# schmidtjonathan/pnmol-experiments

Hardware: AMD Instinct MI355X
Metric: filter steps/sec, 1D heat N=512 nu=2 (white-noise EK1 predict+update) (higher is better)
Workload: dtype f64; 1 GPU; 1-D heat equation, N=512 mesh, IWP(nu=2) EK1, Dirichlet, dt=2^-7, one problem per GPU (kappa sweep), D=1536, m=514; steps_in_one_call=4975, valid=True, problems_per_gpu=1

## Files before the change

### include/pnmol_hip.h

```cpp
#ifndef PNMOL_HIP_H
#define PNMOL_HIP_H

#ifdef __cplusplus
extern "C" {
#endif

typedef struct pnmol_ctx pnmol_ctx;
typedef struct pnmol_filter pnmol_filter;
typedef struct pnmol_state pnmol_state;
typedef struct pnmol_samples pnmol_samples;
typedef struct pnmol_bridge pnmol_bridge;

int pnmol_abi_version(void);
int pnmol_device_count(int* count);
int pnmol_ctx_create(int device, pnmol_ctx** out);
int pnmol_ctx_destroy(pnmol_ctx* ctx);
int pnmol_ctx_synchronize(pnmol_ctx* ctx);
const char* pnmol_last_error(pnmol_ctx* ctx);

int pnmol_fd_solve_batched(pnmol_ctx* ctx, const double* gram_nss, const double* lk_ns, const double* llk_n, int N, int s,
                           double* weights_ns, double* uncertainty_n);
int pnmol_cholesky_lower(pnmol_ctx* ctx, const double* A_nn, int n, double* L_nn);

typedef struct pnmol_filter_desc {
    int d;
    int num_derivatives;
    int nB;
    const double* L;
    const double* B;
    const double* E_sqrtm;
    const double* R_sqrtm;
    const double* Gamma;
    int d_state;
    int dtype;
    const double* K;
} pnmol_filter_desc;

int pnmol_filter_create(pnmol_ctx* ctx, const pnmol_filter_desc* desc, pnmol_filter** out);
int pnmol_filter_destroy(pnmol_filter* f);
int pnmol_filter_sweep_layout(const pnmol_filter* f, int* kernel, int* xcd_home);

int pnmol_filter_set_error_model(pnmol_filter* f, double dt, const double* Sq_inv,
                                 const double* Sq_diag);
int pnmol_filter_prepare_error_model(pnmol_filter* f, double dt);

int pnmol_filter_predict_mean(pnmol_filter* f, const pnmol_state* in, double dt, double* m_at_d);
int pnmol_filter_set_operator(pnmol_filter* f, const double* M_dds, const double* shift_d);
int pnmol_filter_set_operator_diagonal(pnmol_filter* f, const double* jdiag_d, const double* shift_d);

#define PNMOL_REACTION_MAXDEG 7
typedef struct pnmol_reaction {
    int deg_p, deg_a, deg_b;
    double p[PNMOL_REACTION_MAXDEG + 1], a[PNMOL_REACTION_MAXDEG + 1], b[PNMOL_REACTION_MAXDEG + 1];
} pnmol_reaction;
int pnmol_filter_set_reaction(pnmol_filter* f, const pnmol_reaction* r);
int pnmol_filter_linearize(pnmol_filter* f, const pnmol_state* in, double dt);

#define PNMOL_SYSTEM_MAXCOMP  4
#define PNMOL_SYSTEM_MAXTERMS 8
typedef struct pnmol_monomial    { double coef; int pow[PNMOL_SYSTEM_MAXCOMP]; } pnmol_monomial;
typedef struct pnmol_system_poly { int nterms; pnmol_monomial term[PNMOL_SYSTEM_MAXTERMS]; } pnmol_system_poly;
typedef struct pnmol_reaction_system {
    int ncomp;
// ... 82 lines not shown
```

### pnmol-experiments_amd/csrc/pnmol_hip.hip

```cpp
#include <hip/hip_runtime.h>

#include <algorithm>
#include <chrono>
#include <cmath>
#include <cstdio>
#include <cstdlib>
#include <cstring>
#include <string>
#include <utility>
#include <atomic>
#include <vector>

#include "pnmol_hip.h"
#include "pnmol_internal.hpp"

namespace {

constexpr int TLD = NB + 1;
typedef double d4 __attribute__((ext_vector_type(4)));

struct MeasModel {
    const int* ell_col;
    const double* ell_val;
    int w, d, m, dp, mp;
    double c0, c1;
};

constexpr int HW = 4;

struct HRow {
    int idx[HW + 1];
    double cf[HW + 1];
};

__device__ __forceinline__ void h_row_load(const MeasModel& mm, int i, HRow& r) {
    r.idx[0] = (i < mm.d) ? mm.dp + i : 0;
    r.cf[0] = (i < mm.d) ? mm.c1 : 0.0;
// ... 1675 lines not shown
                    L.seen[0] = got;
                }
                __syncthreads();
                const int got = L.seen[0];
                if (got < 0) break;
                if (got == 0) continue;
                ksplit_partial(L.sP[w], Xh, F + ((long)t * NB + fr) * ld + 8 * fk, 0, kh, ld, w, l);
                __syncthreads();
                double* hs = hs_scratch + ((long)H * CB + t) * NB * NB;
#pragma unroll
                for (int r = 0; r < 4; ++r)
                    wt_st(&hs[(wr * 16 + fk + 4 * r) * NB + colC],
                          (L.sP[0][offC + 4 * r * TLD] + L.sP[1][offC + 4 * r * TLD]) +
                              (L.sP[2][offC + 4 * r * TLD] + L.sP[3][offC + 4 * r * TLD]));
                drain_vmem();
                __syncthreads();
                if (tid == 0) flag_st(cl, 2);
            }
        }
    }
}

constexpr int RL_REP = 8;
constexpr int S_SPLIT_FROM = 11, S_SPLIT_H = 9;
__host__ __device__ inline int s_split_count(int CB, bool xl) { return (xl && CB > S_SPLIT_FROM) ? CB - S_SPLIT_FROM : 0; }
constexpr int W_SPLIT_H = 11;
#ifndef PNMOL_W_SPLIT
#define PNMOL_W_SPLIT 0
#endif
__host__ __device__ inline int w_split_count(int RT, int CB) {
    const int RBW = RT - 2 * CB - 1;
    return (PNMOL_W_SPLIT && RBW > 0 && CB > W_SPLIT_H + 1) ? RBW : 0;
}
struct RlFlags {
    int frow, fabort, fxcc, ffeed, fdiag, fnew, fcol, fdiagL, fnewL, frowL, CBp, total;
};
__host__ __device__ inline RlFlags rl_flags(int RT, int CB) {
    const int RTp = (RT + 31) / 32 * 32, CBp = (CB + 31) / 32 * 32;
    RlFlags f;
    f.CBp = CBp;
    f.frow = 0;
    f.fabort = RTp;
    f.fxcc = RTp + 16;
    f.ffeed = RTp + 32;
    f.fdiag = f.ffeed + CBp;
    f.fnew = f.fdiag + RL_REP * CBp;
    f.fcol = f.fnew + RL_REP * CBp;
    f.fdiagL = f.fcol + RL_REP * CBp;
    f.fnewL = f.fdiagL + CBp;
    f.frowL = f.fnewL + CBp;
    f.total = f.frowL + CBp;
    return f;
}
__device__ __forceinline__ int xcc_id() { return __builtin_amdgcn_s_getreg((3 << 11) | 20) & 15; }
struct WaveWait {
    bool dead;
// ... 287 lines not shown
                TileRegs tx;
                tile_regs_from_lds(tx, C.sX, l);
                tile_regs_store<0>(tx, rF, orgX, ld, l);
                drain_vmem();
                if (l == 0) l2_flag_st(rflags, fl.fnewL + J, 1);
                tile_regs_store<16>(tl, rlinv, (unsigned)(J * NB * NB * 8), NB, l);
                tile_regs_store<16>(tx, rF, orgX, ld, l);
                drain_vmem();
                if (l < RL_REP) flag_st(fdiag_all + l * CBp + J, 1);
                if (l < RL_REP) flag_st(fnew_all + l * CBp + J, 1);
            } else {
                wt_rows_from_lds<8>(rF, orgX, ld, C.sX, 0, l);
                drain_vmem();
                if (l < RL_REP) flag_st(fnew_all + l * CBp + J, 1);
            }
        }
    }
    if (w == 2)
        diag4_output(&C.d4[(CB - 1) & 1], l, F + ((long)(CB - 1) * NB) * ld + (long)(CB - 1) * NB, ld, info, (CB - 1) * NB,
                     C.sd[(CB - 1) & 1], smax, pivtol);
    if (l == 0 && ww.dead) atomicMin(info, -2);
}

template <int N, bool FUSED, int MAXT, bool XL>
__global__ __launch_bounds__(256) void k_sweep_rl(const double* __restrict__ G, double* F, double* Linv, int ld, int CB,
                                                  int RT, int* flags, int* info_base, const int* __restrict__ ctr,
                                                  DowndateArgs dd, double* feed, int lenient, int home) {
    __shared__ __attribute__((aligned(16))) union {
        SweepLds L;
        ChainLds C;
    } lds;
    SweepLds& L = lds.L;
    __shared__ __attribute__((aligned(16))) double bulk_ring[4][RING + 2][16 * NB];
    const int tid = threadIdx.x, l = tid & 63, w = __builtin_amdgcn_readfirstlane(tid >> 6);
    const int wr = w >> 1, wc = w & 1, fr = l & 15, fk = l >> 4;
    const RlFlags fl = rl_flags(RT, CB);
    int* frow = flags + fl.frow;
    int* fabort = flags + fl.fabort;
    int* ffeed = flags + fl.ffeed;
    const int* fdiag = flags + fl.fdiag + (blockIdx.x % RL_REP) * fl.CBp;
    const int* fnew = flags + fl.fnew + (blockIdx.x % RL_REP) * fl.CBp;
    const int* fcol = flags + fl.fcol + (blockIdx.x % RL_REP) * fl.CBp;
    int* info = info_base + (*ctr - 1);
    const int bx = XL ? (int)blockIdx.x - home : (int)blockIdx.x;
    if (bx < 0) return;
    if (bx == 0) {
        sweep_chain_role<XL>(lds.C, G, F, Linv, ld, CB, flags, fl, info, feed, lenient, tid, l, w);
        return;
    }
    int I, part = 0;
    if constexpr (XL) {
        const int nsplit = s_split_count(CB, true);
        const int b = bx, nslot = 8 * (CB - 1 + nsplit) + 1;
        if (b < nslot) {
            if (b % 8 != 0) return;
            const int sidx = b / 8;
            if (sidx < CB) {
                I = sidx;
                part = (nsplit > 0 && I >= S_SPLIT_FROM) ? 1 : 0;
            } else {
                I = S_SPLIT_FROM + (sidx - CB);
                part = 2;
            }
        } else {
            if (b % 8 == 0) return;
            const int q = b - nslot;
            I = CB + q - (q + 1) / 8;
        }
    } else {
        I = bx - 1;
    }
#ifdef PNMOL_SWEEP_STAMP
    if (tid == 0) L.stamp_id = part == 1 ? 200 + I : 1 + I;
#endif
    {
        const int zb = RT - CB - 1;
        if (I >= CB && I <= zb) I = (I == CB) ? zb : I - 1;
    }
    const int nwsplit = w_split_count(RT, CB);
    if (I >= RT && I < RT + nwsplit) {
        I = CB + (I - RT);
        part = 2;
    } else if (I >= RT) {
        I -= nwsplit;
        if constexpr (FUSED) {
            if (tid == 0) {
                L.dead = 0, L.seen[0] = 0;
                __builtin_amdgcn_fence(__ATOMIC_ACQUIRE, "agent");
            }
            __syncthreads();
            SWEEP_STAMP(0);
            sweep_downdate_role<N, true>(L, dd, F, ld, CB, CB, frow, fabort, info, I - RT, tid, l, w, *ctr - 1);
        }
        return;
    } else if (nwsplit > 0 && I >= CB && I < RT - CB - 1) {
        part = 1;
    }
    const bool chain = I < CB;
    if (chain && I == 0) return;
    if (tid == 0) {
        L.dead = 0, L.pub = 0, L.pubcnt = part == 2 ? 4 * (I < CB ? S_SPLIT_H : W_SPLIT_H) : 0, L.rdiag = 0, L.rnew = 0, L.rcol = 0, L.rzb = 0;
        L.seen[0] = 0;
        __builtin_amdgcn_fence(__ATOMIC_ACQUIRE, "agent");
    }
    __syncthreads();
    SWEEP_STAMP(0);

    const long rowC = (long)I * NB + wr * 16 + fk;
    const int colC = wc * 16 + fr;
    const int offC = (wr * 16 + fk) * TLD + colC;
    const bool feeds = chain && part != 1;
    const int hsplit = chain ? S_SPLIT_H : W_SPLIT_H;
    const int t0 = part == 2 ? hsplit : 0;
    const int last = part == 1 ? hsplit - 1 : (chain ? I - 2 : CB - 1);
    const int ntiles = part == 1 ? hsplit : (chain ? I : CB);
    d4 n[MAXT];
#pragma unroll
    for (int t = 0; t < MAXT; ++t)
        if (t0 + t < ntiles) {
#pragma unroll
            for (int r = 0; r < 4; ++r) n[t][r] = -G[(rowC + 4 * r) * ld + (long)(t0 + t) * NB + colC];
        }
    d4 accD = {0, 0, 0, 0};
    if (feeds) {
#pragma unroll
        for (int r = 0; r < 4; ++r) {
            const int rl = wr * 16 + fk + 4 * r, cl = colC;
            accD[r] = -G[((long)I * NB + (rl >= cl ? rl : cl)) * ld + (long)I * NB + (rl >= cl ? cl : rl)];
        }
    }
    WaveWait ww{false};
    int known_diag = 0, known_new = 0, known_col = 0;
    const __amdgpu_buffer_rsrc_t rF = wt_rsrc(F), rfeed = wt_rsrc(feed), rflags = wt_rsrc(flags);
    const double* ringw = &bulk_ring[w][0][0];
    const unsigned ring0 = __builtin_amdgcn_readfirstlane((unsigned)(size_t)ringw);
    int roff[4], roffL[4];
#pragma unroll
    for (int c = 0; c < 4; ++c) {
        const int row = 4 * c + (l >> 4);
        roff[c] = (wc * 16 + row) * ld + 2 * ((l & 15) ^ row);
        roffL[c] = (wc * 16 + row) * NB + 2 * ((l & 15) ^ row);
    }
#ifndef PNMOL_EAGER_TILES
#define PNMOL_EAGER_TILES 6
#endif
    constexpr int EAGER_TILES = PNMOL_EAGER_TILES;
    bool pre_b0 = false;
    if constexpr (FUSED) {
        const int RBW = RT - 2 * CB - 1, zb = CB + RBW;
        if (!chain && I > zb) {
            double bq[8] = {0, 0, 0, 0, 0, 0, 0, 0};
            if (dd.va.Sqinv != nullptr) rows8_dot(dd.va.Sqinv, (long)(I - zb - 1) * NB + 8 * w, ld, dd.va.z, bq, l);
            if (l == 0) {
#pragma unroll
                for (int q = 0; q < 8; ++q) L.sd[8 * w + q] = bq[q];
            }
        }
    }
    bool local = false;
    if constexpr (XL) {
        if (chain) {
            if (tid == 0) {
                int v = 0;
                for (int spins = 0; spins < 4096 && (v = flag_ld(flags + fl.fxcc)) == 0; ++spins) __builtin_amdgcn_s_sleep(1);
                L.seen[0] = (v == 1 + xcc_id());
            }
            __syncthreads();
            local = L.seen[0] != 0;
            if (local) fdiag = flags + fl.fdiagL, fnew = flags + fl.fnewL;
        }
    }
    Frag8 ax;
    auto flag_tile = [&](int t) {
        drain_vmem();
        int lastw = 0;
        if (l == 0) lastw = __hip_atomic_fetch_add(&L.pubcnt, 1, __ATOMIC_RELAXED, __HIP_MEMORY_SCOPE_WORKGROUP) == 4 * t + 3;
        if (__builtin_amdgcn_readfirstlane(lastw)) {
            if (l == 0) flag_st(frow + I, t + 1);
            if (XL && chain && l == 0) {
                if (local) l2_flag_st(rflags, fl.frowL + I, t + 1);
                else flag_st(flags + fl.frowL + I, t + 1);
            }
            if (chain && l < RL_REP)
                __hip_atomic_fetch_add(flags + fl.fcol + l * fl.CBp + t, 1, __ATOMIC_RELAXED, __HIP_MEMORY_SCOPE_AGENT);
        }
    };
    if (part == 2) {
        const int* fsrc = (XL && local) ? flags + fl.frowL : frow;
        for (int k = 0; k < t0; ++k) {
            if (chain) {
                if (k + 1 < t0) {
                    relay_progress_min(fsrc + t0, I - t0 + 1, k + 1, known_col, &L.rcol, fabort, ww, w, l);
                } else {
                    relay_progress(fnew, CB - 1, [](int) { return 1; }, t0, known_new, &L.rnew, fabort, ww, w, l);
                    relay_progress_min(fsrc + t0 + 1, I - t0, t0, known_col, &L.rcol, fabort, ww, w, l);
                }
            } else {
                relay_progress(fnew, CB - 1, [](int) { return 1; }, k + 1, known_new, &L.rnew, fabort, ww, w, l);
                relay_progress(fcol, CB - 1, [CB](int q) { return CB - 2 - q; }, k + 1, known_col, &L.rcol, fabort, ww, w, l);
                relay_wait_ge(frow + I, k + 1, &L.rzb, k + 1, fabort, ww, w);
            }
            Frag8 bx;
            frag_ld(ax, F + ((long)I * NB + wr * 16 + fr) * ld + (long)k * NB + 8 * fk);
            frag_ld(bx, F + ((long)I * NB + wc * 16 + fr) * ld + (long)k * NB + 8 * fk);
#pragma unroll
            for (int u0 = 0; u0 < 8; u0 += 4) {
                Frag8 b[4];
#pragma unroll
                for (int q = 0; q < 4; ++q)
                    if (t0 + u0 + q < ntiles)
                        frag_ld(b[q], F + ((long)(t0 + u0 + q) * NB + wc * 16 + fr) * ld + (long)k * NB + 8 * fk);
#pragma unroll
                for (int q = 0; q < 4; ++q)
                    if (t0 + u0 + q < ntiles) {
#pragma unroll
                        for (int s = 0; s < 8; ++s)
                            n[u0 + q] = __builtin_amdgcn_mfma_f64_16x16x4f64(ax.v[s], b[q].v[s], n[u0 + q], 0, 0, 0);
                    }
            }
            if (chain) {
#pragma unroll
                for (int s = 0; s < 8; ++s) accD = __builtin_amdgcn_mfma_f64_16x16x4f64(ax.v[s], bx.v[s], accD, 0, 0, 0);
            }
// ... 642 lines not shown
inline bool fused_loop(const pnmol_filter* f) {
    return f->sweep_mode == 2 && f->n <= 3 && f->fuse_predict != 0 && !f->has_reaction;
}

inline bool sweep_rl_enabled() {
    static const int on = [] {
        const char* e = std::getenv("PNMOL_HIP_SWEEP_RL");
        return e ? std::atoi(e) : 1;
    }();
    return on != 0;
}
inline int sweep_xl_mode() {
    static const int mode = [] {
        const char* e = std::getenv("PNMOL_HIP_SWEEP_XL");
        return e ? (std::atoi(e) != 0 ? 1 : 0) : -1;
    }();
    return mode;
}
constexpr int MAX_DEVICES = 64;
std::atomic<int> live_rl_filters[MAX_DEVICES];
template <int N, bool FUSED>
void launch_sweep(unsigned grid, hipStream_t st, const double* G, double* F, double* Linv, int ld, int CB, int RT, int* flags,
                  int* info, const int* ctr, const DowndateArgs& dd, int* claim, double* hs, int lenient, int home,
                  bool wskip = false) {
    const bool xl = home >= 0;
    const unsigned rgrid = grid + (unsigned)w_split_count(RT, CB);
    unsigned xgrid = 8u * (unsigned)(CB - 1 + s_split_count(CB, true)) + 1u;
    for (unsigned left = rgrid - (unsigned)CB; left > 0; ++xgrid)
        if (xgrid % 8u != 0u) --left;
    xgrid += (unsigned)(xl ? home : 0);
    if (sweep_rl_enabled() && CB <= 9) {
        if (xl) k_sweep_rl<N, FUSED, 9, true><<<xgrid, 256, 0, st>>>(G, F, Linv, ld, CB, RT, flags, info, ctr, dd, hs, lenient, home);
        else k_sweep_rl<N, FUSED, 9, false><<<rgrid + 1, 256, 0, st>>>(G, F, Linv, ld, CB, RT, flags, info, ctr, dd, hs, lenient, home);
    } else if (sweep_rl_enabled() && CB <= 17) {
        if (xl) k_sweep_rl<N, FUSED, 17, true><<<xgrid, 256, 0, st>>>(G, F, Linv, ld, CB, RT, flags, info, ctr, dd, hs, lenient, home);
        else k_sweep_rl<N, FUSED, 17, false><<<rgrid + 1, 256, 0, st>>>(G, F, Linv, ld, CB, RT, flags, info, ctr, dd, hs, lenient, home);
    }
    else
        k_sweep<N, FUSED><<<grid, 256, 0, st>>>(G, F, Linv, ld, CB, RT, flags, info, ctr, dd, claim, hs, lenient, wskip ? 1 : 0);
}

inline bool short_last_panel() {
    static const int on = [] {
        const char* e = std::getenv("PNMOL_HIP_SHORT_LAST");
        return e ? std::atoi(e) : 1;
    }();
    return on != 0;
}
template <int N>
int launch_step(pnmol_filter* f, const double* Pin, const double* min, double frame_dt, double dt, double* Pout,
                double* mout, double* varout, bool record, StepKind kind) {
    pnmol_ctx* ctx = f->ctx;
    hipStream_t st = ctx->stream;
    IwpConsts c = f->iwp;
    for (int a = 0; a < f->n; ++a) {
        const double so = frame_dt == 0.0 ? 1.0 : nordsieck_scale(f->nu, a, frame_dt);
        c.ts[a] = so / nordsieck_scale(f->nu, a, dt);
    }
    MeasModel mm{f->ell_col, f->ell_val, f->ellw, f->d, f->m, f->dp, f->mp,
// ... 8 lines not shown
        if (f->ellw > HW && f->sweep_mode != 0) {
            k_front<<<dim3((mp + 255) / 256, (unsigned)Dp), 256, 0, st>>>(f->Ppred, f->G, f->rdiag, f->Rdense, mm, Dp, f->p32);
            k_front_s<<<dim3((mp + 255) / 256, (unsigned)mp), 256, 0, st>>>(f->G, f->rdiag, f->Rdense, mm);
        } else {
            k_front<<<dim3((mp + 255) / 256, (unsigned)(Dp + mp + (f->sweep_mode == 0 ? mp : 0))), 256, 0, st>>>(
                f->Ppred, f->G, f->rdiag, f->Rdense, mm, Dp, f->p32);
        }
    }
    const long rowI0 = (long)mp + Dp + NB;
    const double* W = f->F + (long)mp * mp;
    const bool have_sq = (f->Sqinv != nullptr && f->sq_dt == dt);
    VecArgs va{f->mpred, f->F + ((long)mp + Dp) * mp, f->F + rowI0 * mp, f->zbuf, have_sq ? f->Sqinv : nullptr,
               mout, f->part};
    const int nreal = f->m - NB * (f->CB - 1);
    DowndateArgs dd{f->Ppred, Pout, varout, dp, 0, va, kind == STEP_FULL ? nullptr : f->Ppred, f->Kg, f->last_ctr, {}, {}, f->p32,
                    (nreal < 8 && short_last_panel()) ? nreal : 0};
    std::memcpy(dd.A1, f->iwp.A1, sizeof(dd.A1));
    std::memcpy(dd.Q1, f->iwp.Q1, sizeof(dd.Q1));
    if (f->sweep_mode == 2) {
        const int t32 = dp / NB, pairs = t32 * (t32 + 1) / 2;
        dd.vrows = 0;
        if constexpr (N <= 3)
            launch_sweep<N, true>(f->RT + pairs, st, f->G, f->F, f->Linv, mp, f->CB, f->RT, f->flags, f->info, f->ctr, dd,
                                  f->flags + f->RT + f->CB + 1, f->hs_scratch, f->p32 ? 2 : 0, f->xcd_home);
    } else {
        if (f->sweep_mode == 1) {
            if (f->w_gemm) {
                launch_sweep<N, false>(2 * f->CB + 1, st, f->G, f->F, f->Linv, mp, f->CB, f->RT, f->flags, f->info, f->ctr, dd,
                                       f->flags + f->RT + f->CB + 1, f->hs_scratch, f->p32 ? 2 : 0, f->xcd_home, true);
                const int nI = (int)(Dp / BDT), nt = nI * (mp / BDT);
                k_w_gemm<<<8 * ((nt + 7) / 8), 256, 0, st>>>(f->G + (long)mp * mp, f->F + rowI0 * mp, f->F + (long)mp * mp, mp, nI, nt);
            } else
            launch_sweep<N, false>(f->RT, st, f->G, f->F, f->Linv, mp, f->CB, f->RT, f->flags, f->info, f->ctr, dd,
                                   f->flags + f->RT + f->CB + 1, f->hs_scratch, f->p32 ? 2 : 0, f->xcd_home);
        } else {
            k_diag0<<<1, 128, 0, st>>>(f->G, f->F, f->Linv, mp, f->info, f->sdiag, f->ctr);
            for (int j = 0; j < f->CB; ++j) {
                const int nrb = f->RT - (j + 1);
                const int ncb = f->CB - 1 - j > 0 ? f->CB - 1 - j : 1;
                k_panel<<<dim3(nrb, ncb), 256, 0, st>>>(f->G, f->F, f->Linv, mp, j, f->CB, f->RBS, f->info, f->sdiag, f->ctr);
            }
        }
        const int tiles = dp / 16;
        const int vrows = (int)(((Dp + mp + 3) / 4 + tiles - 1) / tiles);
        if (f->dd_big) {
            const int T = (int)(Dp / BDT), nt = T * (T + 1) / 2;
            if (f->p32)
// ... 538 lines not shown
    if (const char* gc = std::getenv("PNMOL_HIP_GRAPH_CHUNK")) f->graph_chunk = std::atoi(gc) / 2 * 2;
    if (const char* e = std::getenv("PNMOL_HIP_SWEEP")) f->sweep_mode = std::atoi(e);
    if (f->sweep_mode == 2 && n > 3) f->sweep_mode = 1;
    {
        const char* e = std::getenv("PNMOL_HIP_DD_BIG");
        const bool fits = f->Dp % BDT == 0 && f->mp % BDK == 0 && f->sweep_mode >= 1 && (!f->p32 || f->sweep_mode == 2);
        const bool want = e ? std::atoi(e) != 0 : (f->Dp >= 8192 && f->CB > 17);
        if (fits && want) {
            f->dd_big = 1;
            f->sweep_mode = 1;
            const char* g = std::getenv("PNMOL_HIP_W_GEMM");
            f->w_gemm = (g ? std::atoi(g) != 0 : 1) && f->mp % BDT == 0 && f->CB > 17;
        }
    }
    {
        static std::atomic<int> next_home[MAX_DEVICES];
        const bool rl = sweep_rl_enabled() && f->CB <= 17 && f->sweep_mode >= 1;
        if (rl) {
            const int dv = ctx->device % MAX_DEVICES;
            const int others = live_rl_filters[dv].fetch_add(1);
            f->counted = true;
            const bool xl = sweep_xl_mode() < 0 ? others == 0 : sweep_xl_mode() == 1;
            f->xcd_home = xl ? next_home[dv].fetch_add(1) % 8 : -1;
        }
    }
    FCHK(hipMalloc(&f->sdiag, sizeof(double) * (mp + 1)));
    f->nflags = std::max({f->RT + f->CB + 1 + f->CB * f->CB, rl_flags(f->RT, f->CB).total,
                          rl_flags((int)(f->Dp / NB) + 1, (int)(f->Dp / NB) + 1).total});
    FCHK(hipMalloc(&f->flags, sizeof(int) * f->nflags));
    FCHK(hipMemset(f->flags, 0, sizeof(int) * f->nflags));
    FCHK(hipMalloc(&f->hs_scratch, sizeof(double) * (size_t)std::max(f->CB * f->CB, 2 * f->CB + 2) * NB * NB));
    if (const char* e = std::getenv("PNMOL_HIP_FUSE_PREDICT")) f->fuse_predict = std::atoi(e);
    FCHK(hipMalloc(&f->last_ctr, sizeof(int)));
    FCHK(hipMemset(f->last_ctr, 0, sizeof(int)));
    FCHK(hipMalloc(&f->tickets, sizeof(int)));
    FCHK(hipMemset(f->tickets, 0, sizeof(int)));
    if (f->p32 && f->sweep_mode != 2 && !f->dd_big) {
        ctx->err = "pnmol_filter_create: dtype = fp32 covariance needs the fused sweep (num_derivatives <= 2, PNMOL_HIP_SWEEP unset)";
        return fail(-1);
    }
    FCHK(hipMemcpy(f->ell_col, ecol.data(), sizeof(int) * ecol.size(), hipMemcpyHostToDevice));
    FCHK(hipMemcpy(f->ell_val, eval.data(), sizeof(double) * eval.size(), hipMemcpyHostToDevice));
    {
        std::vector<int> slot((size_t)mp, 0);
        f->base_has_diag = 1;
        for (int i = 0; i < d; ++i) {
// ... 69 lines not shown
    pnmol_dense_free_ws(f);
    pnmol_observe_free_ws(f);
    pnmol_reaction_free_ws(f);
    if (f->ev0) hipEventDestroy(f->ev0);
    if (f->ev1) hipEventDestroy(f->ev1);
    delete f;
    return 0;
}

int pnmol_filter_dims(const pnmol_filter* f, int* d, int* n, int* m, int* dp, int* mp) {
    if (!f) return -1;
    if (d) *d = f->d;
    if (n) *n = f->n;
    if (m) *m = f->m;
    if (dp) *dp = f->dp;
    if (mp) *mp = f->mp;
    return 0;
}

int pnmol_filter_sweep_layout(const pnmol_filter* f, int* kernel, int* xcd_home) {
    if (!f) return -1;
    if (kernel) *kernel = f->sweep_mode == 0 ? 0 : (sweep_rl_enabled() && f->CB <= 17 ? 2 : 1);
    if (xcd_home) *xcd_home = f->xcd_home;
    return 0;
}

int pnmol_filter_set_error_model(pnmol_filter* f, double dt, const double* Sq_inv, const double* Sq_diag) {
    if (!f || !Sq_inv || !Sq_diag || !(dt > 0.0)) return -1;
    pnmol_ctx* ctx = f->ctx;
    HIPCHK(ctx, hipSetDevice(ctx->device));
    const int m = f->m, mp = f->mp;
    std::vector<double> pad((size_t)mp * mp, 0.0);
    for (int i = 0; i < m; ++i) std::memcpy(&pad[(size_t)i * mp], Sq_inv + (size_t)i * m, sizeof(double) * m);
    HIPCHK(ctx, hipStreamSynchronize(ctx->stream));
    if (!f->Sqinv) HIPCHK(ctx, hipMalloc(&f->Sqinv, sizeof(double) * pad.size()));
    HIPCHK(ctx, hipMemcpy(f->Sqinv, pad.data(), sizeof(double) * pad.size(), hipMemcpyHostToDevice));
    f->sqdiag.assign(Sq_diag, Sq_diag + m);
    f->sq_dt = dt;
    drop_graphs(f);
    return 0;
}

int pnmol_filter_prepare_error_model(pnmol_filter* f, double dt) {
    if (!f || !(dt > 0.0)) return -1;
    pnmol_ctx* ctx = f->ctx;
    HIPCHK(ctx, hipSetDevice(ctx->device));
// ... 619 lines not shown
```

### pnmol-experiments_amd/csrc/pnmol_internal.hpp

```cpp
#pragma once
#include <hip/hip_runtime.h>

#include <algorithm>
#include <atomic>
#include <cmath>
#include <string>
#include <vector>

#include "pnmol_hip.h"

constexpr int NB = 32;
constexpr int MAXN = 4;

namespace {
struct IwpConsts {
    double A1[MAXN * MAXN];
    double Q1[MAXN * MAXN];
    double ts[MAXN];
};
}

#define HIPCHK(ctx, call)                                                                        \
    do {                                                                                         \
        hipError_t e__ = (call);                                                                 \
// ... 35 lines not shown
    int qp = 0;
    SweepWs sweep;
    double* dev = nullptr;
    std::vector<double> host;
};

struct pnmol_filter {
    pnmol_ctx* ctx = nullptr;
    int d = 0, n = 0, nu = 0, nB = 0, m = 0, dp = 0, mp = 0, CB = 0, RBS = 0, RBW = 0, RT = 0, ellw = 0;
    int* tickets = nullptr;
    int* last_ctr = nullptr;
    int fuse_predict = 1;
    int* flags = nullptr;
    int nflags = 0;
    double* hs_scratch = nullptr;
    int w_gemm = 0;
    int dd_big = 0;
    int sweep_mode = 2;
    int ds = 0;
    bool counted = false;
    bool registered = false;
    std::atomic<int> states{0};
    int xcd_home = -1;
    int p32 = 0;
    size_t psz = 8;
    long Dp = 0;
    IwpConsts iwp{};
    int* ell_col = nullptr;
    double* ell_val = nullptr;
    int* ell_col_base = nullptr;
    double* ell_val_base = nullptr;
    int* ell_diag_slot = nullptr;
    int base_w = 0, base_has_diag = 0;
    int ell_is_base = 1;
    double* h_op = nullptr;
    double* h_op_dev = nullptr;
    hipEvent_t ev_op = nullptr;
    double *Kg = nullptr, *rdiag = nullptr, *Rdense = nullptr, *shift = nullptr;
    double *G = nullptr, *F = nullptr, *Linv = nullptr, *Ppred = nullptr, *mpred = nullptr, *zbuf = nullptr;
    double *var = nullptr, *Sqinv = nullptr, *rec = nullptr, *part = nullptr, *sdiag = nullptr;
    int* info = nullptr;
    std::vector<double> sqdiag;
    double* Qfull = nullptr;
    int* one = nullptr;
    int* info_err = nullptr;
    double sq_dt = -1.0;
// ... 156 lines not shown
```

### pnmol-experiments_amd/pnmol/_hip.py

```python

import ctypes
import os
import pathlib

import numpy as np


_c_double_p = ctypes.POINTER(ctypes.c_double)
_HERE = pathlib.Path(__file__).resolve().parent
LIB_PATH = pathlib.Path(os.environ.get("PNMOL_HIP_LIB", _HERE.parent / "lib" / "libpnmol_hip.so"))


class PnmolHipError(RuntimeError):
    """A call into libpnmol_hip.so failed."""


class StepOut(ctypes.Structure):
    _fields_ = [
        ("t_new", ctypes.c_double),
        ("diffusion_squared_local", ctypes.c_double),
        ("sigma2_whitened", ctypes.c_double),
        ("error_sigma2", ctypes.c_double),
        ("info", ctypes.c_int),
    ]
# ... 69 lines not shown
    "pnmol_samples_create": (ctypes.c_int, [_vp, ctypes.c_int, ctypes.POINTER(_vp)]),
    "pnmol_samples_destroy": (ctypes.c_int, [_vp]),
    "pnmol_samples_draw": (ctypes.c_int, [_vp, _vp, _c_double_p, ctypes.c_ulonglong, ctypes.c_ulonglong, ctypes.c_double]),
    "pnmol_samples_step_back": (ctypes.c_int, [_vp, _vp, ctypes.c_double, _c_double_p, ctypes.c_ulonglong, ctypes.c_ulonglong,
                                               ctypes.c_double]),
    "pnmol_samples_interpolate": (ctypes.c_int, [_vp, _vp, _vp, ctypes.c_double, _c_double_p, ctypes.c_ulonglong,
                                                 ctypes.c_ulonglong, ctypes.c_double]),
    "pnmol_samples_clone": (ctypes.c_int, [_vp, ctypes.POINTER(_vp)]),
    "pnmol_samples_get": (ctypes.c_int, [_vp, _c_double_p]),
    "pnmol_samples_get_time": (ctypes.c_int, [_vp, _c_double_p]),
    "pnmol_sample_noise": (ctypes.c_int, [_vp, ctypes.c_ulonglong, ctypes.c_ulonglong, ctypes.c_int, ctypes.c_int,
                                          _c_double_p]),
    "pnmol_filter_steps": (ctypes.c_int, [_vp, _vp, ctypes.c_int, ctypes.c_double, _c_double_p, _c_double_p,
                                          ctypes.POINTER(StepOut)]),
    "pnmol_filter_steps_begin": (ctypes.c_int, [_vp, _vp, ctypes.c_int, ctypes.c_double]),
    "pnmol_filter_steps_end": (ctypes.c_int, [_vp, _vp, _c_double_p, _c_double_p, ctypes.POINTER(StepOut)]),
    "pnmol_filter_prepare_steps": (ctypes.c_int, [_vp, _vp, ctypes.c_int, ctypes.c_double]),
    "pnmol_filter_last_steps_ms": (ctypes.c_int, [_vp, ctypes.POINTER(ctypes.c_float)]),
    "pnmol_filter_prepare_error_model": (ctypes.c_int, [_vp, ctypes.c_double]),
    "pnmol_filter_debug_read": (ctypes.c_int, [_vp, ctypes.c_int, _c_double_p, ctypes.c_long]),
    "pnmol_filter_debug_poison": (ctypes.c_int, [_vp]),
    "pnmol_filter_dims": (ctypes.c_int, [_vp] + [ctypes.POINTER(ctypes.c_int)] * 5),
    "pnmol_filter_sweep_layout": (ctypes.c_int, [_vp] + [ctypes.POINTER(ctypes.c_int)] * 2),
    "pnmol_qr_r": (ctypes.c_int, [_vp, _c_double_p, ctypes.c_int, ctypes.c_int, _c_double_p]),
    "pnmol_qr_last_ms": (ctypes.c_int, [ctypes.POINTER(ctypes.c_float)]),
    "pnmol_sqrt_propagate_cholesky_factor": (ctypes.c_int, [_vp, _c_double_p, ctypes.c_int, ctypes.c_int, _c_double_p,
                                                             ctypes.c_int, _c_double_p]),
    "pnmol_sqrt_update": (ctypes.c_int, [_vp, _c_double_p, ctypes.c_int, ctypes.c_int, _c_double_p, _c_double_p,
                                         _c_double_p, _c_double_p, _c_double_p]),
    "pnmol_sqrt_filter_create": (ctypes.c_int, [_vp, ctypes.POINTER(FilterDesc), ctypes.POINTER(_vp)]),
    "pnmol_sqrt_filter_destroy": (ctypes.c_int, [_vp]),
    "pnmol_sqrt_filter_set_state": (ctypes.c_int, [_vp, ctypes.c_double, _c_double_p, _c_double_p]),
    "pnmol_sqrt_filter_get_state": (ctypes.c_int, [_vp, _c_double_p, _c_double_p, _c_double_p]),
    "pnmol_sqrt_filter_predict_mean": (ctypes.c_int, [_vp, ctypes.c_double, _c_double_p]),
    "pnmol_sqrt_filter_set_operator": (ctypes.c_int, [_vp, _c_double_p, _c_double_p]),
    "pnmol_sqrt_filter_prepare_error_model": (ctypes.c_int, [_vp, ctypes.c_double]),
    "pnmol_sqrt_filter_step": (ctypes.c_int, [_vp, ctypes.c_double, ctypes.POINTER(StepOut), _c_double_p]),
    "pnmol_sqrt_filter_steps": (ctypes.c_int, [_vp, ctypes.c_int, ctypes.c_double, _c_double_p, _c_double_p,
                                               ctypes.POINTER(StepOut)]),
    "pnmol_sqrt_filter_last_steps_ms": (ctypes.c_int, [_vp, ctypes.POINTER(ctypes.c_float)]),
    "pnmol_sqrt_update_no_meascov": (ctypes.c_int, [_vp, _c_double_p, ctypes.c_int, ctypes.c_int, _c_double_p,
                                                    _c_double_p, _c_double_p, _c_double_p]),
}

_lib = None


def load_library():
    global _lib
    if _lib is None:
        if not LIB_PATH.exists():
            raise PnmolHipError(
                f"{LIB_PATH} not found: build it with `python __graft_entry__.py` (hipcc --offload-arch=gfx950). "
                "pnmol has no CPU fallback for the filter step."
            )
        lib = ctypes.CDLL(str(LIB_PATH))
        for name, (res, args) in SYMBOLS.items():
            fn = getattr(lib, name)
            fn.restype, fn.argtypes = res, args
        _lib = lib
    return _lib


def _dp(a):
    return a.ctypes.data_as(_c_double_p)


def _f64(a, shape=None):
    a = np.ascontiguousarray(np.asarray(a, dtype=np.float64))
    if shape is not None and a.shape != shape:
        raise ValueError(f"expected shape {shape}, got {a.shape}")
    return a


class Context:

    _cache = {}

    def __init__(self, device=0):
        self.lib = load_library()
# ... 119 lines not shown
        self._live_samples = {}
        self._live_bridges = {}

    def __del__(self):
        live = getattr(self, "_live", None)
        while live:
            _, sh = live.popitem()
            self.lib.pnmol_state_destroy(sh)
        live = getattr(self, "_live_samples", None)
        while live:
            _, sh = live.popitem()
            self.lib.pnmol_samples_destroy(sh)
        live = getattr(self, "_live_bridges", None)
        while live:
            _, sh = live.popitem()
            self.lib.pnmol_bridge_destroy(sh)
        h, self.handle = getattr(self, "handle", None), None
        if h:
            self.lib.pnmol_filter_destroy(h)

    def sweep_layout(self):
        k, x = ctypes.c_int(0), ctypes.c_int(0)
        self.lib.pnmol_filter_sweep_layout(self.handle, ctypes.byref(k), ctypes.byref(x))
        return {"kernel": ("per_panel", "k_sweep", "k_sweep_rl")[k.value], "xcd_home": x.value}

    def dims(self):
        v = [ctypes.c_int(0) for _ in range(5)]
        self.lib.pnmol_filter_dims(self.handle, *[ctypes.byref(x) for x in v])
        return dict(zip(("d", "n", "m", "dp", "mp"), (x.value for x in v)))

    def prepare_error_model(self, dt):
        self.ctx.check(self.lib.pnmol_filter_prepare_error_model(self.handle, float(dt)), "pnmol_filter_prepare_error_model")
        self.error_model_dt = float(dt)

    def set_error_model(self, dt, Sq_inv, Sq_diag):
        a, b = _f64(Sq_inv, (self.m, self.m)), _f64(Sq_diag, (self.m,))
        self.ctx.check(self.lib.pnmol_filter_set_error_model(self.handle, float(dt), _dp(a), _dp(b)),
                       "pnmol_filter_set_error_model")
        self.error_model_dt = float(dt)

    def new_state(self):
        return State(self)

    def new_samples(self, num_samples):
        return Samples(self, num_samples)

    def predict_mean(self, state_in, dt):
# ... 367 lines not shown
```

Baseline: 7940 steps/s.

## Add paired W-tail sweep roles and skip leading zero tiles in bottom rows

Moves the sweep block-to-role mapping into a shared layout header and adds an optional tail role, where one workgroup handles two trailing W rows beyond a split point h. It also lets rows below the zero band skip their leading structurally-zero tiles, writing zeros directly instead of accumulating them. The tail split is off by default and is enabled by an environment variable. This adds layout complexity and new flag protocols that could deadlock or mis-order if they are wrong.

```diff
diff --git a/include/pnmol_hip.h b/include/pnmol_hip.h
--- a/include/pnmol_hip.h
+++ b/include/pnmol_hip.h
@@ -39,6 +39,7 @@
 int pnmol_filter_create(pnmol_ctx* ctx, const pnmol_filter_desc* desc, pnmol_filter** out);
 int pnmol_filter_destroy(pnmol_filter* f);
 int pnmol_filter_sweep_layout(const pnmol_filter* f, int* kernel, int* xcd_home);
+int pnmol_filter_sweep_tail(const pnmol_filter* f, int* h, int* rows_per_tail, int* tails);
 
 int pnmol_filter_set_error_model(pnmol_filter* f, double dt, const double* Sq_inv,
                                  const double* Sq_diag);
diff --git a/pnmol-experiments_amd/csrc/pnmol_hip.hip b/pnmol-experiments_amd/csrc/pnmol_hip.hip
--- a/pnmol-experiments_amd/csrc/pnmol_hip.hip
+++ b/pnmol-experiments_amd/csrc/pnmol_hip.hip
@@ -13,6 +13,7 @@
 
 #include "pnmol_hip.h"
 #include "pnmol_internal.hpp"
+#include "pnmol_sweep_layout.hpp"
 
 namespace {
 
@@ -1734,16 +1735,6 @@
 }
 
 constexpr int RL_REP = 8;
-constexpr int S_SPLIT_FROM = 11, S_SPLIT_H = 9;
-__host__ __device__ inline int s_split_count(int CB, bool xl) { return (xl && CB > S_SPLIT_FROM) ? CB - S_SPLIT_FROM : 0; }
-constexpr int W_SPLIT_H = 11;
-#ifndef PNMOL_W_SPLIT
-#define PNMOL_W_SPLIT 0
-#endif
-__host__ __device__ inline int w_split_count(int RT, int CB) {
-    const int RBW = RT - 2 * CB - 1;
-    return (PNMOL_W_SPLIT && RBW > 0 && CB > W_SPLIT_H + 1) ? RBW : 0;
-}
 struct RlFlags {
     int frow, fabort, fxcc, ffeed, fdiag, fnew, fcol, fdiagL, fnewL, frowL, CBp, total;
 };
@@ -2077,10 +2068,165 @@
     if (l == 0 && ww.dead) atomicMin(info, -2);
 }
 
+template <int TT>
+__device__ __forceinline__ void sweep_tail_role(SweepLds& L, const double* __restrict__ G, double* F, const double* Linv, int ld,
+                                                int CB, int RT, int* flags, const RlFlags& fl, const int* fdiag, const int* fnew,
+                                                const int* fcol, int* info, const VecArgs& va, int h, int I0, int I1, int tid,
+                                                int l, int w) {
+    int* frow = flags + fl.frow;
+    int* fabort = flags + fl.fabort;
+    const int wr = w >> 1, wc = w & 1, fr = l & 15, fk = l >> 4;
+    const int colC = wc * 16 + fr, offC = (wr * 16 + fk) * TLD + colC;
+    const bool two = I1 >= 0;
+    const int IB = two ? I1 : I0;
+    const int zb = RT - CB - 1, nt = CB - h;
+    d4 nA[TT], nB[TT];
+#pragma unroll
+    for (int u = 0; u < TT; ++u)
+        if (u < nt) {
+#pragma unroll
+            for (int r = 0; r < 4; ++r) {
+                nA[u][r] = -G[((long)I0 * NB + wr * 16 + fk + 4 * r) * ld + (long)(h + u) * NB + colC];
+                nB[u][r] = -G[((long)IB * NB + wr * 16 + fk + 4 * r) * ld + (long)(h + u) * NB + colC];
+            }
+        }
+    for (int rr = 0; rr < 2; ++rr) {
+        const int Ir = rr ? IB : I0;
+        if (Ir > zb) {
+            double bq[8] = {0, 0, 0, 0, 0, 0, 0, 0};
+            if (va.Sqinv != nullptr) rows8_dot(va.Sqinv, (long)(Ir - zb - 1) * NB + 8 * w, ld, va.z, bq, l);
+            if (l == 0) {
+#pragma unroll
+                for (int q = 0; q < 8; ++q) L.sP[1][32 * rr + 8 * w + q] = bq[q];
+            }
+        }
+    }
+    WaveWait ww{false};
+    int known_diag = 0, known_new = 0, known_col = 0;
+    const __amdgpu_buffer_rsrc_t rF = wt_rsrc(F);
+    for (int k = 0; k < h; ++k) {
+        relay_progress(fnew, CB - 1, [](int) { return 1; }, k + 1, known_new, &L.rnew, fabort, ww, w, l);
+        relay_progress(fcol, CB - 1, [CB](int q) { return CB - 2 - q; }, k + 1, known_col, &L.rcol, fabort, ww, w, l);
+        relay_wait_ge(frow + I0, k + 1, &L.rzb, 2 * k + 1, fabort, ww, w);
+        relay_wait_ge(frow + IB, k + 1, &L.rzb, 2 * k + 2, fabort, ww, w);
+        Frag8 a0, a1;
+        frag_ld(a0, F + ((long)I0 * NB + wr * 16 + fr) * ld + (long)k * NB + 8 * fk);
+        frag_ld(a1, F + ((long)IB * NB + wr * 16 + fr) * ld + (long)k * NB + 8 * fk);
+#pragma unroll
+        for (int u0 = 0; u0 < TT; u0 += 4) {
+            Frag8 b[4];
+#pragma unroll
+            for (int q = 0; q < 4; ++q)
+                if (u0 + q < nt) frag_ld(b[q], F + ((long)(h + u0 + q) * NB + wc * 16 + fr) * ld + (long)k * NB + 8 * fk);
+#pragma unroll
+            for (int q = 0; q < 4; ++q)
+                if (u0 + q < nt) {
+#pragma unroll
+                    for (int s = 0; s < 8; ++s)
+                        nA[u0 + q] = __builtin_amdgcn_mfma_f64_16x16x4f64(a0.v[s], b[q].v[s], nA[u0 + q], 0, 0, 0);
+#pragma unroll
+                    for (int s = 0; s < 8; ++s)
+                        nB[u0 + q] = __builtin_amdgcn_mfma_f64_16x16x4f64(a1.v[s], b[q].v[s], nB[u0 + q], 0, 0, 0);
+                    mfma_result_guard();
+                }
+        }
+        mfma_result_guard();
+    }
+    auto flag_tile = [&](int t) {
+        drain_vmem();
+        int lastw = 0;
+        if (l == 0) lastw = __hip_atomic_fetch_add(&L.pubcnt, 1, __ATOMIC_RELAXED, __HIP_MEMORY_SCOPE_WORKGROUP) == 4 * t + 3;
+        if (__builtin_amdgcn_readfirstlane(lastw) && l == 0) {
+            flag_st(frow + I0, t + 1);
+            if (two) flag_st(frow + I1, t + 1);
+        }
+    };
+#pragma unroll
+    for (int r = 0; r < 4; ++r) {
+        L.sS[0][offC + 4 * r * TLD] = -nA[0][r];
+        L.sS[1][offC + 4 * r * TLD] = -nB[0][r];
+    }
+    __syncthreads();
+    for (int j = h; j < CB; ++j) {
+        relay_progress(fdiag, CB, [](int) { return 1; }, j + 1, known_diag, &L.rdiag, fabort, ww, w, l);
+        Frag8 bl;
+        frag_ld(bl, Linv + (long)j * NB * NB + (wc * 16 + fr) * NB + 8 * fk);
+        d4 x0 = {0, 0, 0, 0}, x1 = {0, 0, 0, 0};
+#pragma unroll
+        for (int s = 0; s < 8; ++s)
+            x0 = __builtin_amdgcn_mfma_f64_16x16x4f64(L.sS[0][(wr * 16 + fr) * TLD + 8 * fk + s], bl.v[s], x0, 0, 0, 0);
+#pragma unroll
+        for (int s = 0; s < 8; ++s)
+            x1 = __builtin_amdgcn_mfma_f64_16x16x4f64(L.sS[1][(wr * 16 + fr) * TLD + 8 * fk + s], bl.v[s], x1, 0, 0, 0);
+        mfma_result_guard();
+#pragma unroll
+        for (int r = 0; r < 4; ++r) {
+            L.sX[offC + 4 * r * TLD] = x0[r];
+            L.sP[0][offC + 4 * r * TLD] = x1[r];
+        }
+        __syncthreads();
+        wt_rows_from_lds<2>(rF, (unsigned)((((long)I0 * NB) * ld + (long)j * NB) * 8), ld, L.sX, 8 * w, l);
+        if (two) wt_rows_from_lds<2>(rF, (unsigned)((((long)I1 * NB) * ld + (long)j * NB) * 8), ld, L.sP[0], 8 * w, l);
+        const int cnt = CB - 1 - j;
+        if (cnt > 0) {
+            Frag8 a0, a1;
+#pragma unroll
+            for (int s = 0; s < 8; ++s) {
+                a0.v[s] = L.sX[(wr * 16 + fr) * TLD + 8 * fk + s];
+                a1.v[s] = L.sP[0][(wr * 16 + fr) * TLD + 8 * fk + s];
+            }
+            relay_progress(fnew, CB - 1, [](int) { return 1; }, j + 1, known_new, &L.rnew, fabort, ww, w, l);
+            relay_progress(fcol, CB - 1, [CB](int q) { return CB - 2 - q; }, j + 1, known_col, &L.rcol, fabort, ww, w, l);
+            const double* Lt = F + (long)j * NB + ((long)j * NB + wc * 16 + fr) * ld + 8 * fk;
+#pragma unroll
+            for (int u0 = 1; u0 < TT; u0 += 4) {
+                Frag8 b[4];
+#pragma unroll
+                for (int q = 0; q < 4; ++q)
+                    if (u0 + q < TT && u0 + q <= cnt) frag_ld(b[q], Lt + (long)(u0 + q) * NB * ld);
+                if (u0 == 1) flag_tile(j);
+#pragma unroll
+                for (int q = 0; q < 4; ++q)
+                    if (u0 + q < TT && u0 + q <= cnt) {
+                        d4 ea = nA[u0 + q], eb = nB[u0 + q];
+#pragma unroll
+                        for (int s = 0; s < 8; ++s) ea = __builtin_amdgcn_mfma_f64_16x16x4f64(a0.v[s], b[q].v[s], ea, 0, 0, 0);
+#pragma unroll
+                        for (int s = 0; s < 8; ++s) eb = __builtin_amdgcn_mfma_f64_16x16x4f64(a1.v[s], b[q].v[s], eb, 0, 0, 0);
+                        mfma_result_guard();
+                        nA[u0 + q - 1] = ea;
+                        nB[u0 + q - 1] = eb;
+                    }
+            }
+#pragma unroll
+            for (int r = 0; r < 4; ++r) {
+                L.sS[0][offC + 4 * r * TLD] = -nA[0][r];
+                L.sS[1][offC + 4 * r * TLD] = -nB[0][r];
+            }
+            __syncthreads();
+        }
+    }
+    flag_tile(CB - 1);
+    __syncthreads();
+    relay_wait_ge(frow + zb, CB, &L.rzb, 1 << 24, fabort, ww, w);
+    const long Dp = (long)(RT - 2 * CB - 1) * NB;
+    const double* W = F + (long)ld * ld;
+    SWEEP_STAMP(2);
+    for (int rr = 0; rr < (two ? 2 : 1); ++rr) {
+        const int Ir = rr ? I1 : I0;
+        if (Ir == zb) continue;
+        const long row0 = (Ir < zb ? (long)(Ir - CB) * NB : Dp + (long)(Ir - zb - 1) * NB) + 8 * w;
+        vecops_rows8(va, W, ld, Dp, row0, L.sP[1] + 32 * rr + 8 * w, l);
+    }
+    if (l == 0 && ww.dead) atomicMin(info, -2);
+    SWEEP_STAMP(5);
+}
+
 template <int N, bool FUSED, int MAXT, bool XL>
 __global__ __launch_bounds__(256) void k_sweep_rl(const double* __restrict__ G, double* F, double* Linv, int ld, int CB,
                                                   int RT, int* flags, int* info_base, const int* __restrict__ ctr,
-                                                  DowndateArgs dd, double* feed, int lenient, int home) {
+                                                  DowndateArgs dd, double* feed, int lenient, int home, int wtail_h,
+                                                  int pairs) {
     __shared__ __attribute__((aligned(16))) union {
         SweepLds L;
         ChainLds C;
@@ -2103,41 +2249,16 @@
         sweep_chain_role<XL>(lds.C, G, F, Linv, ld, CB, flags, fl, info, feed, lenient, tid, l, w);
         return;
     }
-    int I, part = 0;
-    if constexpr (XL) {
-        const int nsplit = s_split_count(CB, true);
-        const int b = bx, nslot = 8 * (CB - 1 + nsplit) + 1;
-        if (b < nslot) {
-            if (b % 8 != 0) return;
-            const int sidx = b / 8;
-            if (sidx < CB) {
-                I = sidx;
-                part = (nsplit > 0 && I >= S_SPLIT_FROM) ? 1 : 0;
-            } else {
-                I = S_SPLIT_FROM + (sidx - CB);
-                part = 2;
-            }
-        } else {
-            if (b % 8 == 0) return;
-            const int q = b - nslot;
-            I = CB + q - (q + 1) / 8;
-        }
-    } else {
-        I = bx - 1;
-    }
+    const SweepRole role = sweep_role(bx, CB, RT, pairs, XL, wtail_h);
+    if (role.kind == 0) return;
+    const int I = role.I, part = role.part;
 #ifdef PNMOL_SWEEP_STAMP
-    if (tid == 0) L.stamp_id = part == 1 ? 200 + I : 1 + I;
+    {
+        const int zbs = RT - CB - 1, pos = (I >= CB && I <= zbs) ? (I == zbs ? CB : I + 1) : I;
+        if (tid == 0) L.stamp_id = role.kind == 3 ? 224 + (I - CB) / 2 : (role.kind == 4 ? 1 + RT + I : (part == 1 && I < CB ? 200 + I : 1 + pos));
+    }
 #endif
-    {
-        const int zb = RT - CB - 1;
-        if (I >= CB && I <= zb) I = (I == CB) ? zb : I - 1;
-    }
-    const int nwsplit = w_split_count(RT, CB);
-    if (I >= RT && I < RT + nwsplit) {
-        I = CB + (I - RT);
-        part = 2;
-    } else if (I >= RT) {
-        I -= nwsplit;
+    if (role.kind == 4) {
         if constexpr (FUSED) {
             if (tid == 0) {
                 L.dead = 0, L.seen[0] = 0;
@@ -2145,16 +2266,30 @@
             }
             __syncthreads();
             SWEEP_STAMP(0);
-            sweep_downdate_role<N, true>(L, dd, F, ld, CB, CB, frow, fabort, info, I - RT, tid, l, w, *ctr - 1);
+            sweep_downdate_role<N, true>(L, dd, F, ld, CB, CB, frow, fabort, info, I, tid, l, w, *ctr - 1);
         }
         return;
-    } else if (nwsplit > 0 && I >= CB && I < RT - CB - 1) {
-        part = 1;
+    }
+    if (role.kind == 3) {
+        if constexpr (FUSED) {
+            if (tid == 0) {
+                L.dead = 0, L.pubcnt = 4 * wtail_h, L.pub = 4 * wtail_h, L.rdiag = 0, L.rnew = 0, L.rcol = 0, L.rzb = 0;
+                __builtin_amdgcn_fence(__ATOMIC_ACQUIRE, "agent");
+            }
+            __syncthreads();
+            SWEEP_STAMP(0);
+            sweep_tail_role<(MAXT - 1) / 2>(L, G, F, Linv, ld, CB, RT, flags, fl, fdiag, fnew, fcol, info, dd.va, wtail_h, I, role.I2,
+                                            tid, l, w);
+        }
+        return;
     }
     const bool chain = I < CB;
-    if (chain && I == 0) return;
+    const bool feeds = chain && part != 1;
+    const int hsplit = chain ? S_SPLIT_H : wtail_h;
+    const int idq = (FUSED && I > RT - CB - 1) ? I - (RT - CB) : 0;
+    const int t0 = part == 2 ? hsplit : idq;
     if (tid == 0) {
-        L.dead = 0, L.pub = 0, L.pubcnt = part == 2 ? 4 * (I < CB ? S_SPLIT_H : W_SPLIT_H) : 0, L.rdiag = 0, L.rnew = 0, L.rcol = 0, L.rzb = 0;
+        L.dead = 0, L.pub = 0, L.pubcnt = 4 * t0, L.rdiag = 0, L.rnew = 0, L.rcol = 0, L.rzb = 0;
         L.seen[0] = 0;
         __builtin_amdgcn_fence(__ATOMIC_ACQUIRE, "agent");
     }
@@ -2164,9 +2299,18 @@
     const long rowC = (long)I * NB + wr * 16 + fk;
     const int colC = wc * 16 + fr;
     const int offC = (wr * 16 + fk) * TLD + colC;
-    const bool feeds = chain && part != 1;
-    const int hsplit = chain ? S_SPLIT_H : W_SPLIT_H;
-    const int t0 = part == 2 ? hsplit : 0;
+    if (idq > 0) {
+        for (int e = tid; e < NB * TLD; e += 256) L.sP[1][e] = 0.0;
+        __syncthreads();
+        const __amdgpu_buffer_rsrc_t rFz = wt_rsrc(F);
+        for (int t = 0; t < idq; ++t)
+            wt_rows_from_lds<2>(rFz, (unsigned)((((long)I * NB) * ld + (long)t * NB) * 8), ld, L.sP[1], 8 * w, l);
+        if (part == 1) {
+            drain_vmem();
+            __syncthreads();
+            if (tid == 0) flag_st(frow + I, idq);
+        }
+    }
     const int last = part == 1 ? hsplit - 1 : (chain ? I - 2 : CB - 1);
     const int ntiles = part == 1 ? hsplit : (chain ? I : CB);
     d4 n[MAXT];
@@ -2203,7 +2347,7 @@
     bool pre_b0 = false;
     if constexpr (FUSED) {
         const int RBW = RT - 2 * CB - 1, zb = CB + RBW;
-        if (!chain && I > zb) {
+        if (!chain && I > zb && part != 1) {
             double bq[8] = {0, 0, 0, 0, 0, 0, 0, 0};
             if (dd.va.Sqinv != nullptr) rows8_dot(dd.va.Sqinv, (long)(I - zb - 1) * NB + 8 * w, ld, dd.va.z, bq, l);
             if (l == 0) {
@@ -2243,17 +2387,11 @@
     if (part == 2) {
         const int* fsrc = (XL && local) ? flags + fl.frowL : frow;
         for (int k = 0; k < t0; ++k) {
-            if (chain) {
-                if (k + 1 < t0) {
-                    relay_progress_min(fsrc + t0, I - t0 + 1, k + 1, known_col, &L.rcol, fabort, ww, w, l);
-                } else {
-                    relay_progress(fnew, CB - 1, [](int) { return 1; }, t0, known_new, &L.rnew, fabort, ww, w, l);
-                    relay_progress_min(fsrc + t0 + 1, I - t0, t0, known_col, &L.rcol, fabort, ww, w, l);
-                }
+            if (k + 1 < t0) {
+                relay_progress_min(fsrc + t0, I - t0 + 1, k + 1, known_col, &L.rcol, fabort, ww, w, l);
             } else {
-                relay_progress(fnew, CB - 1, [](int) { return 1; }, k + 1, known_new, &L.rnew, fabort, ww, w, l);
-                relay_progress(fcol, CB - 1, [CB](int q) { return CB - 2 - q; }, k + 1, known_col, &L.rcol, fabort, ww, w, l);
-                relay_wait_ge(frow + I, k + 1, &L.rzb, k + 1, fabort, ww, w);
+                relay_progress(fnew, CB - 1, [](int) { return 1; }, t0, known_new, &L.rnew, fabort, ww, w, l);
+                relay_progress_min(fsrc + t0 + 1, I - t0, t0, known_col, &L.rcol, fabort, ww, w, l);
             }
             Frag8 bx;
             frag_ld(ax, F + ((long)I * NB + wr * 16 + fr) * ld + (long)k * NB + 8 * fk);
@@ -2942,19 +3080,16 @@
 template <int N, bool FUSED>
 void launch_sweep(unsigned grid, hipStream_t st, const double* G, double* F, double* Linv, int ld, int CB, int RT, int* flags,
                   int* info, const int* ctr, const DowndateArgs& dd, int* claim, double* hs, int lenient, int home,
-                  bool wskip = false) {
+                  bool wskip = false, int wtail_h = 0) {
     const bool xl = home >= 0;
-    const unsigned rgrid = grid + (unsigned)w_split_count(RT, CB);
-    unsigned xgrid = 8u * (unsigned)(CB - 1 + s_split_count(CB, true)) + 1u;
-    for (unsigned left = rgrid - (unsigned)CB; left > 0; ++xgrid)
-        if (xgrid % 8u != 0u) --left;
-    xgrid += (unsigned)(xl ? home : 0);
+    const int h = FUSED ? wtail_h : 0, pairs = FUSED ? (int)grid - RT : 0;
+    const unsigned g = sweep_grid((int)grid, CB, RT, pairs, xl, h, xl ? home : 0);
     if (sweep_rl_enabled() && CB <= 9) {
-        if (xl) k_sweep_rl<N, FUSED, 9, true><<<xgrid, 256, 0, st>>>(G, F, Linv, ld, CB, RT, flags, info, ctr, dd, hs, lenient, home);
-        else k_sweep_rl<N, FUSED, 9, false><<<rgrid + 1, 256, 0, st>>>(G, F, Linv, ld, CB, RT, flags, info, ctr, dd, hs, lenient, home);
+        if (xl) k_sweep_rl<N, FUSED, 9, true><<<g, 256, 0, st>>>(G, F, Linv, ld, CB, RT, flags, info, ctr, dd, hs, lenient, home, h, pairs);
+        else k_sweep_rl<N, FUSED, 9, false><<<g, 256, 0, st>>>(G, F, Linv, ld, CB, RT, flags, info, ctr, dd, hs, lenient, home, h, pairs);
     } else if (sweep_rl_enabled() && CB <= 17) {
-        if (xl) k_sweep_rl<N, FUSED, 17, true><<<xgrid, 256, 0, st>>>(G, F, Linv, ld, CB, RT, flags, info, ctr, dd, hs, lenient, home);
-        else k_sweep_rl<N, FUSED, 17, false><<<rgrid + 1, 256, 0, st>>>(G, F, Linv, ld, CB, RT, flags, info, ctr, dd, hs, lenient, home);
+        if (xl) k_sweep_rl<N, FUSED, 17, true><<<g, 256, 0, st>>>(G, F, Linv, ld, CB, RT, flags, info, ctr, dd, hs, lenient, home, h, pairs);
+        else k_sweep_rl<N, FUSED, 17, false><<<g, 256, 0, st>>>(G, F, Linv, ld, CB, RT, flags, info, ctr, dd, hs, lenient, home, h, pairs);
     }
     else
         k_sweep<N, FUSED><<<grid, 256, 0, st>>>(G, F, Linv, ld, CB, RT, flags, info, ctr, dd, claim, hs, lenient, wskip ? 1 : 0);
@@ -3009,7 +3144,7 @@
         dd.vrows = 0;
         if constexpr (N <= 3)
             launch_sweep<N, true>(f->RT + pairs, st, f->G, f->F, f->Linv, mp, f->CB, f->RT, f->flags, f->info, f->ctr, dd,
-                                  f->flags + f->RT + f->CB + 1, f->hs_scratch, f->p32 ? 2 : 0, f->xcd_home);
+                                  f->flags + f->RT + f->CB + 1, f->hs_scratch, f->p32 ? 2 : 0, f->xcd_home, false, f->w_tail_h);
     } else {
         if (f->sweep_mode == 1) {
             if (f->w_gemm) {
@@ -3594,6 +3729,12 @@
             f->counted = true;
             const bool xl = sweep_xl_mode() < 0 ? others == 0 : sweep_xl_mode() == 1;
             f->xcd_home = xl ? next_home[dv].fetch_add(1) % 8 : -1;
+            if (f->sweep_mode == 2 && f->RT - 2 * f->CB - 1 > 0 && f->CB >= 2) {
+                const char* e = std::getenv("PNMOL_HIP_W_TAIL");
+                int h = e ? std::atoi(e) : w_tail_default(f->CB, xl);
+                if (h > 0) h = std::max({1, f->CB - w_tail_cap(f->CB), std::min(h, f->CB - 1)});
+                f->w_tail_h = h > 0 ? h : 0;
+            }
         }
     }
     FCHK(hipMalloc(&f->sdiag, sizeof(double) * (mp + 1)));
@@ -3709,6 +3850,15 @@
     if (!f) return -1;
     if (kernel) *kernel = f->sweep_mode == 0 ? 0 : (sweep_rl_enabled() && f->CB <= 17 ? 2 : 1);
     if (xcd_home) *xcd_home = f->xcd_home;
+    return 0;
+}
+
+int pnmol_filter_sweep_tail(const pnmol_filter* f, int* h, int* rows_per_tail, int* tails) {
+    if (!f) return -1;
+    const int ns = w_tail_rows(f->RT, f->CB, f->w_tail_h);
+    if (h) *h = ns > 0 ? f->w_tail_h : 0;
+    if (rows_per_tail) *rows_per_tail = ns > 1 ? 2 : ns;
+    if (tails) *tails = (ns + 1) / 2;
     return 0;
 }
 
diff --git a/pnmol-experiments_amd/csrc/pnmol_internal.hpp b/pnmol-experiments_amd/csrc/pnmol_internal.hpp
--- a/pnmol-experiments_amd/csrc/pnmol_internal.hpp
+++ b/pnmol-experiments_amd/csrc/pnmol_internal.hpp
@@ -81,6 +81,7 @@
     bool registered = false;
     std::atomic<int> states{0};
     int xcd_home = -1;
+    int w_tail_h = 0;
     int p32 = 0;
     size_t psz = 8;
     long Dp = 0;
diff --git a/pnmol-experiments_amd/csrc/pnmol_sweep_layout.hpp b/pnmol-experiments_amd/csrc/pnmol_sweep_layout.hpp
--- /dev/null
+++ b/pnmol-experiments_amd/csrc/pnmol_sweep_layout.hpp
@@ -0,0 +1,76 @@
+#pragma once
+
+#if defined(__HIPCC__)
+#define PNMOL_HD __host__ __device__
+#else
+#define PNMOL_HD
+#endif
+
+constexpr int S_SPLIT_FROM = 11, S_SPLIT_H = 9;
+PNMOL_HD inline int s_split_count(int CB, bool xl) { return (xl && CB > S_SPLIT_FROM) ? CB - S_SPLIT_FROM : 0; }
+PNMOL_HD inline int w_tail_cap(int CB) { return CB <= 9 ? 4 : 8; }
+PNMOL_HD inline int w_tail_default(int CB, bool xl) {
+    (void)CB, (void)xl;
+    return 0;
+}
+PNMOL_HD inline int w_tail_rows(int RT, int CB, int h) {
+    const int RBW = RT - 2 * CB - 1;
+    if (h <= 0 || h >= CB || RBW < 0 || CB - h > w_tail_cap(CB)) return 0;
+    return RBW + 1 + (h < CB - h ? h : CB - h);
+}
+struct SweepRole {
+    int kind, I, part, I2;
+};
+PNMOL_HD inline int sweep_home_moves(int CB, int RT, int pairs, bool xl, int h) {
+    const int ns = w_tail_rows(RT, CB, h);
+    if (!xl || ns == 0) return 0;
+    const int nq = h < CB - h ? h : CB - h;
+    int mv = (RT - CB) + (ns + 1) / 2 + pairs - 224;
+    const int room = 32 - CB - s_split_count(CB, true);
+    mv = mv < room ? mv : room;
+    mv = mv < CB - nq ? mv : CB - nq;
+    return mv > 0 ? mv : 0;
+}
+PNMOL_HD inline SweepRole sweep_role(int b, int CB, int RT, int pairs, bool xl, int h) {
+    const int ns = w_tail_rows(RT, CB, h), ntails = (ns + 1) / 2, zb = RT - CB - 1;
+    if (b < 0) return {0, 0, 0, -1};
+    if (b == 0) return {1, 0, 0, -1};
+    int idx;
+    int nmove = 0;
+    if (xl) {
+        const int nsplit = s_split_count(CB, true);
+        nmove = sweep_home_moves(CB, RT, pairs, true, h);
+        const int nslot = 8 * (CB - 1 + nsplit + nmove) + 1;
+        if (b < nslot) {
+            if (b % 8 != 0) return {0, 0, 0, -1};
+            const int s = b / 8;
+            if (s < CB) return {2, s, (nsplit > 0 && s >= S_SPLIT_FROM) ? 1 : 0, -1};
+            if (s < CB + nsplit) return {2, S_SPLIT_FROM + (s - CB), 2, -1};
+            return {2, RT - nmove + (s - CB - nsplit), 0, -1};
+        }
+        if (b % 8 == 0) return {0, 0, 0, -1};
+        const int q = b - nslot;
+        idx = q - (q + 1) / 8;
+    } else {
+        if (b - 1 < CB) return {b == 1 ? 0 : 2, b - 1, 0, -1};
+        idx = b - 1 - CB;
+    }
+    const int nrows = RT - CB - nmove;
+    if (idx < nrows) {
+        int I = CB + idx;
+        if (I <= zb) I = (I == CB) ? zb : I - 1;
+        return {2, I, (I < CB + ns) ? 1 : 0, -1};
+    }
+    idx -= nrows;
+    if (idx < ntails) return {3, CB + 2 * idx, 0, (2 * idx + 1 < ns) ? CB + 2 * idx + 1 : -1};
+    return {4, idx - ntails, 0, -1};
+}
+PNMOL_HD inline unsigned sweep_grid(int nlog, int CB, int RT, int pairs, bool xl, int h, int home) {
+    const int ntails = (w_tail_rows(RT, CB, h) + 1) / 2;
+    if (!xl) return (unsigned)(nlog + ntails + 1);
+    const int nmove = sweep_home_moves(CB, RT, pairs, true, h);
+    unsigned g = 8u * (unsigned)(CB - 1 + s_split_count(CB, true) + nmove) + 1u;
+    for (int left = nlog - CB - nmove + ntails; left > 0; ++g)
+        if (g % 8u != 0u) --left;
+    return g + (unsigned)home;
+}
diff --git a/pnmol-experiments_amd/pnmol/_hip.py b/pnmol-experiments_amd/pnmol/_hip.py
--- a/pnmol-experiments_amd/pnmol/_hip.py
+++ b/pnmol-experiments_amd/pnmol/_hip.py
@@ -115,6 +115,7 @@
     "pnmol_filter_debug_poison": (ctypes.c_int, [_vp]),
     "pnmol_filter_dims": (ctypes.c_int, [_vp] + [ctypes.POINTER(ctypes.c_int)] * 5),
     "pnmol_filter_sweep_layout": (ctypes.c_int, [_vp] + [ctypes.POINTER(ctypes.c_int)] * 2),
+    "pnmol_filter_sweep_tail": (ctypes.c_int, [_vp] + [ctypes.POINTER(ctypes.c_int)] * 3),
     "pnmol_qr_r": (ctypes.c_int, [_vp, _c_double_p, ctypes.c_int, ctypes.c_int, _c_double_p]),
     "pnmol_qr_last_ms": (ctypes.c_int, [ctypes.POINTER(ctypes.c_float)]),
     "pnmol_sqrt_propagate_cholesky_factor": (ctypes.c_int, [_vp, _c_double_p, ctypes.c_int, ctypes.c_int, _c_double_p,
@@ -135,6 +136,7 @@
     "pnmol_sqrt_update_no_meascov": (ctypes.c_int, [_vp, _c_double_p, ctypes.c_int, ctypes.c_int, _c_double_p,
                                                     _c_double_p, _c_double_p, _c_double_p]),
 }
+OPTIONAL_SYMBOLS = {"pnmol_filter_sweep_tail"}
 
 _lib = None
 
@@ -149,6 +151,8 @@
             )
         lib = ctypes.CDLL(str(LIB_PATH))
         for name, (res, args) in SYMBOLS.items():
+            if name in OPTIONAL_SYMBOLS and not hasattr(lib, name):
+                continue
             fn = getattr(lib, name)
             fn.restype, fn.argtypes = res, args
         _lib = lib
@@ -314,7 +318,12 @@
     def sweep_layout(self):
         k, x = ctypes.c_int(0), ctypes.c_int(0)
         self.lib.pnmol_filter_sweep_layout(self.handle, ctypes.byref(k), ctypes.byref(x))
-        return {"kernel": ("per_panel", "k_sweep", "k_sweep_rl")[k.value], "xcd_home": x.value}
+        out = {"kernel": ("per_panel", "k_sweep", "k_sweep_rl")[k.value], "xcd_home": x.value}
+        if hasattr(self.lib, "pnmol_filter_sweep_tail"):
+            h, r, t = ctypes.c_int(0), ctypes.c_int(0), ctypes.c_int(0)
+            self.lib.pnmol_filter_sweep_tail(self.handle, ctypes.byref(h), ctypes.byref(r), ctypes.byref(t))
+            out["w_tail"] = {"h": h.value, "rows_per_tail": r.value, "tails": t.value}
+        return out
 
     def dims(self):
         v = [ctypes.c_int(0) for _ in range(5)]
```

Result: slower. 7605 steps/s (-4.2%).
